# kwea123/ngp_pl

Measured on AMD Instinct MI355X. Metric: train rays/sec (800x800 Lego-like, 8192 rays/batch/GPU, full step incl. optimizer), higher is better.
Workload: dtype f16/f32

## Files before the change

### ngp_pl_amd/csrc/march.hip

```cpp
#pragma clang fp contract(off)

#include <cstdlib>
#include <chrono>
#include <type_traits>
#include "ngp_common.h"

#define NGP_SQRT3 1.73205080757f

namespace {

__device__ __forceinline__ float2 aabb_hit(float ox, float oy, float oz, float ix, float iy, float iz,
                                           float cx, float cy, float cz, float hx, float hy, float hz) {
    const float tminx = (cx - hx - ox) * ix, tmaxx = (cx + hx - ox) * ix;
    const float tminy = (cy - hy - oy) * iy, tmaxy = (cy + hy - oy) * iy;
    const float tminz = (cz - hz - oz) * iz, tmaxz = (cz + hz - oz) * iz;
    const float t1 = fmaxf(fmaxf(fminf(tminx, tmaxx), fminf(tminy, tmaxy)), fminf(tminz, tmaxz));
    const float t2 = fminf(fminf(fmaxf(tminx, tmaxx), fmaxf(tminy, tmaxy)), fmaxf(tminz, tmaxz));
    if (t1 > t2) return make_float2(-1.0f, -1.0f);
    return make_float2(t1, t2);
}

__device__ __forceinline__ float2 sphere_hit(float ox, float oy, float oz, float dx, float dy, float dz,
                                             float cx, float cy, float cz, float radius) {
    const float cox = ox - cx, coy = oy - cy, coz = oz - cz;
// ... 369 lines not shown
        int k = 1;
        const bool occ = march_probe<SIMPLE>(ray, p, mine, x, y, z, dt, t_next, &k);
        const unsigned long long empty_mask = ~__ballot(occ);
        int chain = occ ? ((lane << 8) | 64) : ((lane << 8) | (lane + k > 64 ? 64 : lane + k));
#pragma unroll 1
        for (int round = 0; round < 6; ++round) {
            const int h = chain & 0xff;
            const bool go = h < 64 && ((empty_mask >> h) & 1ull);
            const int via = __builtin_amdgcn_ds_bpermute((h & 63) << 2, chain);
            if (go) chain = via;
            if (!__ballot(go)) break;
        }
        unsigned long long emit = 0ull;
        float next_pending = -1.0f;
        bool finished = false;
        int v = entry;
        while (v < 64) {
            if (v >= nvalid) { finished = true; break; }
            if ((empty_mask >> v) & 1ull) {
                const int pk = __builtin_amdgcn_readlane(chain, v);
                const int h = pk & 0xff;
                if (h >= 64) {
                    next_pending = __builtin_bit_cast(float, __builtin_amdgcn_readlane(__builtin_bit_cast(int, t_next), pk >> 8));
                    v = 64;
                    break;
                }
                v = h;
                continue;
            }
            const unsigned long long un = empty_mask >> v;
            const int u = un ? v + (int)__builtin_ctzll(un) : 64;
            const int hi = u < nvalid ? u : nvalid;
            if (hi > v) {
                const int len = hi - v;
                emit |= (len >= 64 ? ~0ull : ((1ull << len) - 1ull)) << v;
            }
            if (nvalid < 64 && u >= nvalid) { finished = true; break; }
            v = u;
        }
        const int room = cap - n;
        const bool my = (emit >> lane) & 1ull;
        const int rank = __popcll(emit & ((1ull << lane) - 1ull));
        if (my && rank < room) store(n + rank, mine);
        const int cnt = __popcll(emit);
        n += cnt < room ? cnt : room;
        if (finished || n >= cap) break;
        pending = next_pending;
        if (pending >= 0 && !(pending < t2)) break;
        t_start = t_end;
    }
    return n;
}

struct MarchPrologue { const float* center; const float* half_size; float near_distance; uint32_t seed_lo, seed_hi; float* hits_out; float* noise_out; };
template <bool SIMPLE, bool PROLOGUE>
__global__ void __launch_bounds__(256)
march_train_count_wave_kernel(const float* __restrict__ rays_o, const float* __restrict__ rays_d,
                              const float* __restrict__ hits_t, const float* __restrict__ noise,
                              MarchParams p, int max_samples, int n_rays,
                              int64_t* __restrict__ rays_a, float* __restrict__ t_scratch, int32_t* __restrict__ counts, MarchPrologue pro) {
    const int r = __builtin_amdgcn_readfirstlane((int)((blockIdx.x * blockDim.x + threadIdx.x) >> 6));
    const int lane = threadIdx.x & 63;
    if (r >= n_rays) return;
    const Ray ray = load_ray(rays_o, rays_d, r);
    float t1, t2, jitter;
    if (PROLOGUE) {
        const float2 t = aabb_hit(ray.ox, ray.oy, ray.oz, ray.ix, ray.iy, ray.iz, pro.center[0], pro.center[1], pro.center[2],
                                  pro.half_size[0], pro.half_size[1], pro.half_size[2]);
        t1 = -1.0f; t2 = -1.0f;
        if (t.y > 0) { t1 = fmaxf(t.x, 0.0f); t2 = t.y; }
        if (t1 >= 0 && t1 < pro.near_distance) t1 = pro.near_distance;
        jitter = (float)(ngp_pcg_hash(ngp_rng_key(pro.seed_lo, pro.seed_hi, (uint32_t)r)) >> 8) * (1.0f / 16777216.0f);
        if (lane == 0) { reinterpret_cast<float2*>(pro.hits_out)[r] = make_float2(t1, t2); pro.noise_out[r] = jitter; }
    } else {
        t1 = hits_t[2 * r]; t2 = hits_t[2 * r + 1]; jitter = noise[r];
    }
    if (t1 >= 0) t1 = fmaf(calc_dt(t1, p), jitter, t1);
    float* __restrict__ row = t_scratch + (size_t)r * max_samples;
    int n = 0;
    if (t1 >= 0) n = march_tile_walk<SIMPLE>(ray, p, t1, t2, max_samples, lane, (unsigned int)r, [row](int i, float t) { row[i] = t; });
    if (lane == 0) {
        rays_a[3 * (size_t)r] = r;
        rays_a[3 * (size_t)r + 2] = n;
        if (counts) counts[r] = n;
    }
}

__global__ void __launch_bounds__(1024)
march_train_scan_kernel(int64_t* __restrict__ rays_a, int n_rays, int32_t* __restrict__ counter, int first_k, int32_t* __restrict__ offs_k) {
    __shared__ int s_wave[16], s_wave_k[16];
    __shared__ int s_carry, s_carry_k;
    const int tid = threadIdx.x;
    if (tid == 0) { s_carry = 0; s_carry_k = 0; }
    __syncthreads();
    for (int base = 0; base < n_rays; base += 8192) {
        const int r0 = base + 8 * tid;
        int v[8];
#pragma unroll
        for (int k = 0; k < 8; ++k) v[k] = (r0 + k < n_rays) ? (int)rays_a[3 * (size_t)(r0 + k) + 2] : 0;
        int run = ngp_block_scan_tile<8>(v, s_wave, &s_carry);
#pragma unroll
        for (int k = 0; k < 8; ++k) {
            if (r0 + k < n_rays) rays_a[3 * (size_t)(r0 + k) + 1] = run;
            run += v[k];
        }
        if (offs_k) {
            int vk[8];
#pragma unroll
            for (int k = 0; k < 8; ++k) vk[k] = min(v[k], first_k);
            int run_k = ngp_block_scan_tile<8>(vk, s_wave_k, &s_carry_k);
#pragma unroll
            for (int k = 0; k < 8; ++k) {
                if (r0 + k < n_rays) offs_k[r0 + k] = run_k;
                run_k += vk[k];
            }
        }
        __syncthreads();
    }
    if (tid == 0) { counter[0] = s_carry; counter[1] = n_rays; if (offs_k) counter[3] = s_carry_k; }
}

__global__ void __launch_bounds__(256)
march_train_write_kernel(const float* __restrict__ rays_o, const float* __restrict__ rays_d,
                         const int64_t* __restrict__ rays_a, const float* __restrict__ t_scratch,
                         MarchParams p, int max_samples, int n_rays,
                         float* __restrict__ xyzs, float* __restrict__ dirs,
                         float* __restrict__ deltas, float* __restrict__ ts,
                         int first_k, int32_t* __restrict__ list_k, int32_t* __restrict__ n_clear,
// ... 444 lines not shown
RenderLayout render_layout(int n_rays, int chunk_scale, float esf) {
    RenderLayout L;
    const int min_samples = (esf == 0.0f) ? 1 : 4;
    const long long R = n_rays;
    L.m_cap = R * (chunk_scale > min_samples ? chunk_scale : min_samples);
    size_t off = 0;
    auto take = [&](size_t bytes) { const size_t o = off; off += (bytes + 255) / 256 * 256; return o; };
    L.hits = take(R * 8); L.alive0 = take(R * 4); L.alive1 = take(R * 4); L.n_eff = take(R * 4); L.offsets = take(R * 4); L.emitted = take(R * 4);
    L.plan = take((RENDER_MAX_ITERS + 1) * sizeof(RenderPlan)); L.total = take(8); L.block_any = take(RENDER_MASK_WORDS * 4);
    const long long slack = 64;
    L.xyzs = take(L.m_cap * 12); L.dirs = take(L.m_cap * 12); L.deltas = take((L.m_cap + slack) * 4); L.ts = take((L.m_cap + slack) * 4);
    L.feats = take(L.m_cap * 64); L.sigmas = take((L.m_cap + slack) * 4); L.rgbs = take((L.m_cap + slack) * 12);
    L.bytes = off;
    return L;
}

struct RenderHost {
    int32_t* counts = nullptr;
    hipEvent_t ev[RENDER_RING] = {};
    int device = -1;
    int init() {
        int dev = 0;
        hipError_t e = hipGetDevice(&dev);
        if (e != hipSuccess) return (int)e;
        if (dev == device) return 0;
        if (device >= 0) {
            for (int i = 0; i < RENDER_RING; ++i) (void)hipEventDestroy(ev[i]);
            (void)hipHostFree(counts);
            device = -1;
        }
        e = hipHostMalloc(reinterpret_cast<void**>(&counts), RENDER_RING * sizeof(int32_t), hipHostMallocDefault);
        if (e != hipSuccess) return (int)e;
        for (int i = 0; i < RENDER_RING; ++i) {
            e = hipEventCreateWithFlags(&ev[i], hipEventDisableTiming);
            if (e != hipSuccess) return (int)e;
        }
        device = dev;
        return 0;
    }
};
thread_local RenderHost g_render_host;
static int g_render_block_hops = 1;
static int g_render_wave_rays = 80000;


double render_wait_limit_s() {
    static const double v = [] { const char* e = getenv("NGP_SPIN_TIMEOUT_S"); const double x = e ? atof(e) : 30.0; return x > 0 ? x : 30.0; }();
    return v;
}

template <typename F> void with_bool(bool flag, F f) { if (flag) f(std::true_type{}); else f(std::false_type{}); }

void launch_train_count(const float* rays_o, const float* rays_d, const float* hits_t, const float* noise, const MarchParams& p, int max_samples,
                        int n_rays, int64_t* rays_a, float* t_scratch, int32_t* counts, const MarchPrologue* pro, ngp_stream_t stream) {
    const dim3 grid(ngp_div_up((long long)n_rays * 64, 256));
    with_bool(p.simple, [&](auto S) { with_bool(pro != nullptr, [&](auto P) {
        hipLaunchKernelGGL((march_train_count_wave_kernel<decltype(S)::value, decltype(P)::value>), grid, dim3(256), 0, ngp_stream(stream),
                           rays_o, rays_d, hits_t, noise, p, max_samples, n_rays, rays_a, t_scratch, counts, pro ? *pro : MarchPrologue{});
    }); });
}

void launch_train_write(const float* rays_o, const float* rays_d, const int64_t* rays_a, const float* t_scratch, float scale, float exp_step_factor,
                        int grid_size, int max_samples, int n_rays, float* xyzs, float* dirs, float* deltas, float* ts,
                        int first_k, int32_t* list_k, int32_t* n_clear, const int32_t* offs_k,
                        const int32_t* counts, int64_t* rays_a_out, int32_t* counter, ngp_stream_t stream) {
    const MarchParams p = make_march_params(nullptr, 1, grid_size, scale, scale, exp_step_factor, max_samples);
    hipLaunchKernelGGL(march_train_write_kernel, dim3(ngp_div_up((long long)n_rays * 64, 256)), dim3(256), 0, ngp_stream(stream),
                       rays_o, rays_d, rays_a, t_scratch, p, max_samples, n_rays, xyzs, dirs, deltas, ts, first_k, list_k, n_clear, offs_k,
                       counts, rays_a_out, counter);
}

}

extern "C" {
#pragma GCC visibility push(default)

int ngp_abi_version(void) { return 6; }

int ngp_march_guard_first(float* probe12) {
    NGP_CHECK_PTR(probe12);
    return (int)hipMemcpyFromSymbol(probe12, HIP_SYMBOL(g_march_guard_first), 12 * sizeof(float), 0, hipMemcpyDeviceToHost);
}

int ngp_march_guard_read(uint32_t* counts4, int reset) {
    NGP_CHECK_PTR(counts4);
    hipError_t e = hipMemcpyFromSymbol(counts4, HIP_SYMBOL(g_march_guard), 4 * sizeof(uint32_t), 0, hipMemcpyDeviceToHost);
    if (e != hipSuccess) return (int)e;
    if (reset) {
        const uint32_t z[4] = {0, 0, 0, 0};
        e = hipMemcpyToSymbol(HIP_SYMBOL(g_march_guard), z, sizeof(z), 0, hipMemcpyHostToDevice);
    }
    return (int)e;
}
const char* ngp_build_arch(void) { return "gfx950"; }

int ngp_ray_aabb_intersect(const float* rays_o, const float* rays_d, const float* centers,
                           const float* half_sizes, int n_rays, int n_voxels, int max_hits,
                           int32_t* hit_cnt, float* hits_t, int64_t* hits_voxel_idx, ngp_stream_t stream) {
    if (n_rays < 0 || n_voxels < 0 || max_hits < 1) return NGP_EINVAL;
    if (n_rays == 0) return 0;
    NGP_CHECK_PTR(rays_o); NGP_CHECK_PTR(rays_d); NGP_CHECK_PTR(hit_cnt); NGP_CHECK_PTR(hits_t); NGP_CHECK_PTR(hits_voxel_idx);
    if (n_voxels > 0) { NGP_CHECK_PTR(centers); NGP_CHECK_PTR(half_sizes); }
    hipLaunchKernelGGL(ray_prim_intersect_kernel<false>, dim3(ngp_div_up(n_rays, 256)), dim3(256), 0, ngp_stream(stream),
                       rays_o, rays_d, centers, half_sizes, n_rays, n_voxels, max_hits, hit_cnt, hits_t, hits_voxel_idx);
    return NGP_LAUNCH_RESULT();
}

int ngp_ray_sphere_intersect(const float* rays_o, const float* rays_d, const float* centers,
                             const float* radii, int n_rays, int n_spheres, int max_hits,
                             int32_t* hit_cnt, float* hits_t, int64_t* hits_sphere_idx, ngp_stream_t stream) {
    if (n_rays < 0 || n_spheres < 0 || max_hits < 1) return NGP_EINVAL;
    if (n_rays == 0) return 0;
    NGP_CHECK_PTR(rays_o); NGP_CHECK_PTR(rays_d); NGP_CHECK_PTR(hit_cnt); NGP_CHECK_PTR(hits_t); NGP_CHECK_PTR(hits_sphere_idx);
    if (n_spheres > 0) { NGP_CHECK_PTR(centers); NGP_CHECK_PTR(radii); }
    hipLaunchKernelGGL(ray_prim_intersect_kernel<true>, dim3(ngp_div_up(n_rays, 256)), dim3(256), 0, ngp_stream(stream),
                       rays_o, rays_d, centers, radii, n_rays, n_spheres, max_hits, hit_cnt, hits_t, hits_sphere_idx);
    return NGP_LAUNCH_RESULT();
}

int ngp_ray_aabb_near(const float* rays_o, const float* rays_d, const float* center,
                      const float* half_size, float near_distance, int n_rays, float* hits_t,
                      ngp_stream_t stream) {
    if (n_rays < 0) return NGP_EINVAL;
    if (n_rays == 0) return 0;
// ... 67 lines not shown
                       density_grid, density_grid_tmp, decay_grid, decay, n_cells, stats);
    return NGP_LAUNCH_RESULT();
}

int ngp_raymarching_train_count(const float* rays_o, const float* rays_d, const float* hits_t,
                                const uint8_t* density_bitfield, int cascades, float scale,
                                float exp_step_factor, const float* noise, int grid_size,
                                int max_samples, int n_rays, int64_t* rays_a, int32_t* counter,
                                float* t_scratch, ngp_stream_t stream) {
    return ngp_raymarching_train_count_k(rays_o, rays_d, hits_t, density_bitfield, cascades, scale, exp_step_factor, noise, grid_size, max_samples,
                                         n_rays, rays_a, counter, t_scratch, 0, nullptr, stream);
}

int ngp_raymarching_train_count_k(const float* rays_o, const float* rays_d, const float* hits_t,
                                  const uint8_t* density_bitfield, int cascades, float scale,
                                  float exp_step_factor, const float* noise, int grid_size,
                                  int max_samples, int n_rays, int64_t* rays_a, int32_t* counter,
                                  float* t_scratch, int first_k, int32_t* offs_k, ngp_stream_t stream) {
    if (n_rays < 0 || cascades < 1 || grid_size < 1 || grid_size > 1024 || max_samples < 1) return NGP_EINVAL;
    if (offs_k != nullptr && (first_k < 1 || first_k > 64)) return NGP_EINVAL;
    NGP_CHECK_PTR(counter);
    if (n_rays > 0) {
        NGP_CHECK_PTR(rays_o); NGP_CHECK_PTR(rays_d); NGP_CHECK_PTR(hits_t); NGP_CHECK_PTR(density_bitfield);
        NGP_CHECK_PTR(noise); NGP_CHECK_PTR(rays_a); NGP_CHECK_PTR(t_scratch);
        const MarchParams p = make_march_params(density_bitfield, cascades, grid_size, scale, scale, exp_step_factor, max_samples);
        launch_train_count(rays_o, rays_d, hits_t, noise, p, max_samples, n_rays, rays_a, t_scratch, nullptr, nullptr, stream);
    }
    hipLaunchKernelGGL(march_train_scan_kernel, dim3(1), dim3(1024), 0, ngp_stream(stream), rays_a, n_rays, counter, first_k, offs_k);
    return NGP_LAUNCH_RESULT();
}

int ngp_raymarching_train_write(const float* rays_o, const float* rays_d, const int64_t* rays_a,
                                const float* t_scratch, float scale, float exp_step_factor,
                                int grid_size, int max_samples, int n_rays,
                                float* xyzs, float* dirs, float* deltas, float* ts, ngp_stream_t stream) {
    if (n_rays < 0 || grid_size < 1 || max_samples < 1) return NGP_EINVAL;
    if (n_rays == 0) return 0;
    NGP_CHECK_PTR(rays_o); NGP_CHECK_PTR(rays_d); NGP_CHECK_PTR(rays_a); NGP_CHECK_PTR(t_scratch);
    launch_train_write(rays_o, rays_d, rays_a, t_scratch, scale, exp_step_factor, grid_size, max_samples, n_rays, xyzs, dirs, deltas, ts,
                       0, nullptr, nullptr, nullptr, nullptr, nullptr, nullptr, stream);
    return NGP_LAUNCH_RESULT();
}

int ngp_march_train_fused(const float* rays_o, const float* rays_d, const float* center, const float* half_size,
                          float near_distance, uint64_t seed, const uint8_t* density_bitfield, int cascades, float scale,
                          float exp_step_factor, int grid_size, int max_samples, int n_rays,
                          float* hits_t, float* noise, int64_t* rays_a, int32_t* counts, int32_t* counter, float* t_scratch,
                          float* xyzs, float* dirs, float* deltas, float* ts, ngp_stream_t stream) {
    if (n_rays < 1 || cascades < 1 || grid_size < 1 || grid_size > 1024 || max_samples < 1) return NGP_EINVAL;
    NGP_CHECK_PTR(rays_o); NGP_CHECK_PTR(rays_d); NGP_CHECK_PTR(center); NGP_CHECK_PTR(half_size); NGP_CHECK_PTR(density_bitfield);
    NGP_CHECK_PTR(hits_t); NGP_CHECK_PTR(noise); NGP_CHECK_PTR(rays_a); NGP_CHECK_PTR(counts); NGP_CHECK_PTR(counter); NGP_CHECK_PTR(t_scratch);
    NGP_CHECK_PTR(xyzs); NGP_CHECK_PTR(dirs); NGP_CHECK_PTR(deltas); NGP_CHECK_PTR(ts);
    if (reinterpret_cast<uintptr_t>(counts) & 15) return NGP_EINVAL;
    const MarchParams p = make_march_params(density_bitfield, cascades, grid_size, scale, scale, exp_step_factor, max_samples);
    const MarchPrologue pro = {center, half_size, near_distance, (uint32_t)seed, (uint32_t)(seed >> 32), hits_t, noise};
    launch_train_count(rays_o, rays_d, nullptr, nullptr, p, max_samples, n_rays, rays_a, t_scratch, counts, &pro, stream);
    launch_train_write(rays_o, rays_d, rays_a, t_scratch, scale, exp_step_factor, grid_size, max_samples, n_rays, xyzs, dirs, deltas, ts,
                       0, nullptr, nullptr, nullptr, counts, rays_a, counter, stream);
    return NGP_LAUNCH_RESULT();
}

int ngp_raymarching_train_write_k(const float* rays_o, const float* rays_d, const int64_t* rays_a,
                                  const float* t_scratch, float scale, float exp_step_factor,
                                  int grid_size, int max_samples, int n_rays,
                                  float* xyzs, float* dirs, float* deltas, float* ts,
                                  int first_k, int32_t* list_k, int32_t* n_clear, ngp_stream_t stream) {
    if (n_rays < 0 || grid_size < 1 || max_samples < 1 || first_k < 1 || first_k > 64) return NGP_EINVAL;
    if (n_rays == 0) return 0;
    NGP_CHECK_PTR(rays_o); NGP_CHECK_PTR(rays_d); NGP_CHECK_PTR(rays_a); NGP_CHECK_PTR(t_scratch); NGP_CHECK_PTR(list_k);
    launch_train_write(rays_o, rays_d, rays_a, t_scratch, scale, exp_step_factor, grid_size, max_samples, n_rays, xyzs, dirs, deltas, ts,
                       first_k, list_k, n_clear, nullptr, nullptr, nullptr, nullptr, stream);
    return NGP_LAUNCH_RESULT();
}

int ngp_raymarching_train_write_kc(const float* rays_o, const float* rays_d, const int64_t* rays_a,
                                   const float* t_scratch, float scale, float exp_step_factor,
                                   int grid_size, int max_samples, int n_rays,
                                   float* xyzs, float* dirs, float* deltas, float* ts,
                                   int first_k, const int32_t* offs_k, int32_t* list_k, int32_t* n_clear, ngp_stream_t stream) {
    if (n_rays < 0 || grid_size < 1 || max_samples < 1 || first_k < 1 || first_k > 64) return NGP_EINVAL;
    if (n_rays == 0) return 0;
    NGP_CHECK_PTR(rays_o); NGP_CHECK_PTR(rays_d); NGP_CHECK_PTR(rays_a); NGP_CHECK_PTR(t_scratch); NGP_CHECK_PTR(list_k); NGP_CHECK_PTR(offs_k);
    launch_train_write(rays_o, rays_d, rays_a, t_scratch, scale, exp_step_factor, grid_size, max_samples, n_rays, xyzs, dirs, deltas, ts,
                       first_k, list_k, n_clear, offs_k, nullptr, nullptr, nullptr, stream);
    return NGP_LAUNCH_RESULT();
}

int ngp_raymarching_test(const float* rays_o, const float* rays_d, float* hits_t,
                         const int64_t* alive_indices, const uint8_t* density_bitfield,
                         int cascades, float scale, float exp_step_factor, int grid_size,
                         int max_samples, int n_samples, int n_alive,
                         float* xyzs, float* dirs, float* deltas, float* ts,
                         int32_t* n_eff_samples, ngp_stream_t stream) {
    if (n_alive < 0 || cascades < 1 || grid_size < 1 || grid_size > 1024 || max_samples < 1 || n_samples < 1) return NGP_EINVAL;
    if (n_alive == 0) return 0;
    NGP_CHECK_PTR(rays_o); NGP_CHECK_PTR(rays_d); NGP_CHECK_PTR(hits_t); NGP_CHECK_PTR(alive_indices);
    NGP_CHECK_PTR(density_bitfield); NGP_CHECK_PTR(xyzs); NGP_CHECK_PTR(dirs); NGP_CHECK_PTR(deltas);
    NGP_CHECK_PTR(ts); NGP_CHECK_PTR(n_eff_samples);
    const MarchParams p = make_march_params(density_bitfield, cascades, grid_size, scale, (float)cascades, exp_step_factor, max_samples);
    with_bool(p.simple, [&](auto S) {
        hipLaunchKernelGGL(march_test_kernel<decltype(S)::value>, dim3(ngp_div_up(n_alive, 64)), dim3(64), 0, ngp_stream(stream),
                           rays_o, rays_d, hits_t, alive_indices, p, n_samples, n_alive, xyzs, dirs, deltas, ts, n_eff_samples);
    });
    return NGP_LAUNCH_RESULT();
}

int ngp_compact_alive(const int64_t* alive_in, const int32_t* n_eff, int n, int64_t* alive_out, int32_t* count,
                      int64_t* total_samples, ngp_stream_t stream) {
    if (n < 0) return NGP_EINVAL;
    if (n == 0) return 0;
    NGP_CHECK_PTR(alive_in); NGP_CHECK_PTR(alive_out); NGP_CHECK_PTR(count);
    hipLaunchKernelGGL(compact_alive_kernel, dim3(ngp_div_up(n, 256)), dim3(256), 0, ngp_stream(stream),
// ... 132 lines not shown
```

### ngp_pl_amd/csrc/ngp_internal.h

```cpp
#ifndef NGP_HIP_INTERNAL_H
#define NGP_HIP_INTERNAL_H
#include "../../include/ngp_hip.h"
#ifdef __cplusplus
extern "C" {
#endif

typedef struct ngp_grid_partials {
    int32_t n_levels, reserved;
    int64_t value_end;
    uint32_t offset[NGP_MAX_LEVELS + 1];
    int32_t k_split[NGP_MAX_LEVELS];
    int64_t part_off[NGP_MAX_LEVELS];
    const float* partial;
} ngp_grid_partials;

int ngp_field_bwd_guarded(const ngp_half* feats, const float* dirs, const ngp_half* h, const ngp_half* density_w,
                          const ngp_half* rgb_w, const float* dL_dsigmas, const float* dL_drgbs, float loss_scale,
                          const float* loss_scale_dev, float din_limit, int n_samples, const int32_t* active_idx, const int32_t* n_active,
                          ngp_half* dh_scratch, ngp_half* dfeats, float* wgrad_partial, int32_t* nonfinite2, int parity,
                          ngp_stream_t stream);
int ngp_adam_use_loss_scaler(float* state, int slot, float growth_factor, float backoff_factor, int growth_interval,
                             float min_scale, float max_scale);
struct ngp_stepper;
int ngp_stepper_before_update(struct ngp_stepper* s, int32_t** found_inf);
// ... 89 lines not shown
int ngp_composite_train_bw_tail(const float* dL_dopacity, const float* dL_ddepth, const float* dL_drgb,
                                const float* dL_dws, const float* sigmas, const float* rgbs, const float* ws,
                                const float* deltas, const float* ts, const int64_t* rays_a,
                                const float* opacity, const float* depth, const float* rgb, float T_threshold,
                                int n_rays, int n_samples, float* dL_dsigmas, float* dL_drgbs,
                                const int32_t* ray_counts, int32_t* active_idx, const float* xyzs, float* x_active,
                                int32_t* n_active, int32_t* n_active_host, float* loss, float* sq_err,
                                const void* workspace, size_t workspace_bytes, ngp_stream_t stream);

int ngp_hashgrid_fwd_list(const float* x, const float* xyz_min, const float* xyz_max,
                          const ngp_half* table, const ngp_grid_meta* meta, int n_samples,
                          const int32_t* list, int n_list_max, const int32_t* n_list_dev,
                          ngp_half* feats, ngp_stream_t stream);

int ngp_field_fwd_list(const ngp_half* feats, const float* dirs,
                       const ngp_half* density_w, const ngp_half* rgb_w, int n_samples,
                       const int32_t* list, int n_list_max, const int32_t* n_list_dev,
                       float* sigmas, float* rgbs, ngp_half* h_out, ngp_stream_t stream);

int ngp_density_fwd_scatter(const ngp_half* feats, const ngp_half* density_w, int n_samples,
                            const int32_t* scatter_idx, float* sigmas_out, ngp_stream_t stream);

int ngp_debug_hashgrid_fwd_map(const ngp_grid_meta* meta, int n_chunks, int32_t* xcd_level_chunk, int max_blocks);

int ngp_debug_render_block_hops(int enabled);

int ngp_debug_render_wave_rays(int max_rays);

int ngp_stepper_two_rounds(const ngp_stepper* s);

int ngp_occupancy_update_workspace_layout(int cascades, int grid_size, size_t* tmp_off, size_t* cell_idx_off, size_t* xyzs_off);

int ngp_feats_to_rowmajor(const ngp_half* feats, int n_levels, int n_samples, ngp_half* out,
                          ngp_stream_t stream);

int ngp_feats_from_rowmajor(const ngp_half* in, int n_levels, int n_samples, ngp_half* feats,
                            ngp_stream_t stream);

int ngp_adam_step_partials(float* param, ngp_half* param_h, const float* partials, int n_partials,
                           float* m, float* v, int n, float lr, float beta1, float beta2, float eps,
                           float weight_decay, int step, float grad_scale, const int32_t* found_inf,
                           ngp_stream_t stream);

int ngp_active_samples(const int64_t* rays_a, const int64_t* total_samples, int n_rays,
                       int32_t* ray_offsets, int32_t* active_idx, int32_t* n_active,
                       ngp_stream_t stream);

int ngp_hashgrid_bwd(const float* x, const float* xyz_min, const float* xyz_max,
                     const ngp_half* dfeats , const ngp_grid_meta* meta,
                     int n_samples, void* grad_table, int grad_is_f32, ngp_stream_t stream);

#ifdef __cplusplus
}
#endif
#endif
```

### ngp_pl_amd/csrc/stepper.hip

```cpp
#include "ngp_common.h"
#include "adam_common.h"
#include "comm.h"
#include <algorithm>
#include <chrono>
#include <cstdlib>
#include <cstring>
#include <new>

namespace {

constexpr int N_MARKS = 9;

double spin_limit_s() {
    static const double v = [] { const char* e = getenv("NGP_SPIN_TIMEOUT_S"); const double x = e ? atof(e) : 30.0; return x > 0 ? x : 30.0; }();
    return v;
}

}

struct ngp_stepper {
    ngp_stepper_config c;
    ngp_step_buffers b;
    hipEvent_t ready[2] = {}, done[2] = {};
    hipEvent_t mark[N_MARKS] = {}, march_t[2][2] = {};
    bool mark_set[N_MARKS] = {}, march_t_set[2] = {};
    int timing = 0;
    int next_set = 0;
    bool has_pending = false;
    const float* pend_o = nullptr; const float* pend_d = nullptr;
    int pend_set = 0;
    uint64_t marches = 0;
    int32_t S = 0, n_part = 0, last_set = 0;
    bool binned = false;
    int device = 0;
    double t_wait = 0.0, t_enqueue = 0.0;
    long long n_fronts = 0;
    const float* next_o = nullptr; const float* next_d = nullptr;
    hipStream_t next_main = nullptr, next_side = nullptr;
    int march_at = 2;
    int two_round_mode = 2, two_round_k = 32;
    bool two_round_active = false, two_rounds = false;
    int set_k[2] = {0, 0};
    long long two_round_steps = 0;
    int32_t prev_S = 0;
    ngp_comm* comm = nullptr;
    ngp_exchange_config x = {};
    hipEvent_t ev_small = nullptr, ev_chunk[8] = {}, ev_done = nullptr;
    hipEvent_t ev_x0 = nullptr, ev_x1 = nullptr, ev_m = nullptr;
    bool x_times_set = false;
    long long tails = 0;
    int64_t group_end[16] = {};
    struct SampleSet { float* xyzs; float* dirs; float* deltas; float* ts; };
    SampleSet samples[2] = {};
    bool two_sample_sets = false;
    bool expanded[2] = {false, false};
    int32_t* counts[2] = {nullptr, nullptr};
    int counts_rays = 0;
    bool same_stream[2] = {false, false};
    int32_t* guard = nullptr;
    int guard_parity = 0;
    bool guard_armed = false;
    bool fused[2] = {false, false};
    float* scaler_state = nullptr;
    bool scaler_on = false;
    int scaler_slot = 0;
    float scaler_growth = 2.0f, scaler_backoff = 0.5f, scaler_lo = 9.5367431640625e-07f , scaler_hi = 1.152921504606847e18f ;
    int scaler_interval = 2000;
};

void destroy_exchange_events(ngp_stepper* s);

namespace {

struct HostTimer {
    double* acc; std::chrono::steady_clock::time_point t0;
    explicit HostTimer(double* a) : acc(a), t0(std::chrono::steady_clock::now()) {}
    ~HostTimer() { *acc += std::chrono::duration<double>(std::chrono::steady_clock::now() - t0).count(); }
};

#define STEP_TRY(expr) do { const int rc_ = (expr); if (rc_ != 0) return rc_; } while (0)
#define STEP_HIP(expr) do { const hipError_t e_ = (expr); if (e_ != hipSuccess) return (int)e_; } while (0)

int check_buffers(const ngp_stepper_config& c, const ngp_step_buffers& b) {
    if (b.n_rays < 1 || b.cap < b.n_rays || b.max_partials < 1) return NGP_EINVAL;
    const void* need[] = {b.xyzs, b.dirs, b.deltas, b.ts, b.feats, b.h, b.sigmas, b.rgbs, b.ws, b.dL_dsigmas, b.dL_drgbs, b.active, b.dh,
                          b.dfeats, b.total, b.opacity, b.depth, b.rgb, b.dL_drgb, b.dL_dopacity, b.ray_offs, b.zeros, b.n_active, b.stats,
                          b.partials, b.fw_ws, b.hits_t[0], b.hits_t[1], b.rays_a[0], b.rays_a[1], b.noise[0], b.noise[1], b.scratch[0],
                          b.scratch[1], b.counter[0], b.counter[1]};
    for (const void* p : need) if (p == nullptr) return NGP_EINVAL;
    if (b.bin_max > 0 && (b.bin_ws == nullptr || b.x_act == nullptr)) return NGP_EINVAL;
    if (b.distortion && (!b.ws_incl || !b.wts_incl || !b.dL_dws || !b.dist || !b.dist_seed)) return NGP_EINVAL;
    if (c.lambda_distortion > 0 && !b.distortion) return NGP_EINVAL;
    return 0;
}

inline void mark(ngp_stepper* s, int i, hipStream_t st) {
    if (!s->timing) return;
    if (hipEventRecord(s->mark[i], st) == hipSuccess) s->mark_set[i] = true;
}

int wait_march(ngp_stepper* s, int k, bool count_is_enough = false) {
    volatile int32_t* cnt = s->b.counter[k];
    const auto t_begin = std::chrono::steady_clock::now();
    struct Account { ngp_stepper* s; std::chrono::steady_clock::time_point t0;
                     ~Account() { const double d = std::chrono::duration<double>(std::chrono::steady_clock::now() - t0).count(); s->t_wait += d; s->t_enqueue -= d; } } account{s, t_begin};
    const auto t_end = t_begin + std::chrono::duration<double>(spin_limit_s());
    unsigned spins = 0;
    while (cnt[0] < 0) {
        if ((++spins & 1023u) == 0) {
            if (hipEventQuery(s->done[k]) == hipSuccess) break;
// ... 10 lines not shown

enum { AT_TOP = 0, AT_HASHGRID_FWD, AT_MLP_FWD, AT_COMPOSITE_FW, AT_COMPOSITE_BW, AT_MLP_BWD, AT_HASHGRID_BWD, AT_ADAM };
int march_at_from_env() {
    static const int v = [] {
        const char* e = getenv("NGP_MARCH_AT");
        if (!e) return (int)AT_MLP_FWD;
        const char* names[] = {"top", "hashgrid_fwd", "mlp_fwd", "composite_fw", "composite_bw", "mlp_bwd", "hashgrid_bwd", "adam"};
        for (int i = 0; i < 8; ++i) if (strcmp(e, names[i]) == 0) return i;
        return (int)AT_MLP_FWD;
    }();
    return v;
}

int ensure_counts(ngp_stepper* s) {
    const int n = s->b.n_rays;
    if (s->counts[0] != nullptr && s->counts_rays >= n) return 0;
    for (int k = 0; k < 2; ++k) { if (s->counts[k]) (void)hipFree(s->counts[k]); s->counts[k] = nullptr; }
    for (int k = 0; k < 2; ++k) STEP_HIP(hipMalloc(reinterpret_cast<void**>(&s->counts[k]), ((size_t)n + 8) * sizeof(int32_t)));
    s->counts_rays = n;
    return 0;
}

int do_march(ngp_stepper* s, const float* rays_o, const float* rays_d, hipStream_t main, hipStream_t side);
inline int march_next_if_at(ngp_stepper* s, int stage) {
    if (s->next_o == nullptr || s->march_at != stage) return 0;
    const float* o = s->next_o; const float* d = s->next_d;
    s->next_o = s->next_d = nullptr;
    return do_march(s, o, d, s->next_main, s->next_side);
}

int do_march(ngp_stepper* s, const float* rays_o, const float* rays_d, hipStream_t main, hipStream_t side) {
    if (s->has_pending) return NGP_EINVAL;
    NGP_CHECK_PTR(rays_o); NGP_CHECK_PTR(rays_d);
    const ngp_stepper_config& c = s->c;
    const ngp_step_buffers& b = s->b;
    const int k = s->next_set; s->next_set ^= 1;
    if (side != main) {
        STEP_HIP(hipEventRecord(s->ready[k], main));
        STEP_HIP(hipStreamWaitEvent(side, s->ready[k], 0));
    }
    b.counter[k][0] = -1;
    b.counter[k][3] = -1;
    s->march_t_set[k] = false;
    s->same_stream[k] = side == main;
    s->fused[k] = false;
    if (s->timing) STEP_HIP(hipEventRecord(s->march_t[k][0], side));
    const bool lists_wanted = (s->two_round_mode == 1 || (s->two_round_mode == 2 && s->two_round_active)) && b.list_k && b.list_rest &&
                              b.two_round_counts && b.offs_k[k];
    constexpr int FUSED_MARCH_MAX_RAYS = 32768;
    if (s->two_sample_sets && !lists_wanted && b.n_rays <= FUSED_MARCH_MAX_RAYS) {
        STEP_TRY(ensure_counts(s));
        const ngp_stepper::SampleSet& w = s->samples[k];
        s->set_k[k] = 0;
        STEP_TRY(ngp_march_train_fused(rays_o, rays_d, c.center, c.half_size, c.near_distance, c.noise_seed + 0x9E3779B97F4A7C15ull * (++s->marches),
                                       c.density_bitfield, c.cascades, c.scale, c.exp_step_factor, c.grid_size, c.max_samples, b.n_rays,
                                       b.hits_t[k], b.noise[k], b.rays_a[k], s->counts[k], b.counter[k], b.scratch[k],
                                       w.xyzs, w.dirs, w.deltas, w.ts, (ngp_stream_t)side));
        s->expanded[k] = true;
        s->fused[k] = true;
        if (s->timing) { STEP_HIP(hipEventRecord(s->march_t[k][1], side)); s->march_t_set[k] = true; }
        STEP_HIP(hipEventRecord(s->done[k], side));
        s->has_pending = true; s->pend_o = rays_o; s->pend_d = rays_d; s->pend_set = k;
        return 0;
    }
    STEP_TRY(ngp_ray_aabb_near_noise(rays_o, rays_d, c.center, c.half_size, c.near_distance, b.n_rays, c.noise_seed + 0x9E3779B97F4A7C15ull * (++s->marches),
                                     b.hits_t[k], b.noise[k], (ngp_stream_t)side));
    const bool lists = (s->two_round_mode == 1 || (s->two_round_mode == 2 && s->two_round_active)) && b.list_k && b.list_rest &&
                       b.two_round_counts && b.offs_k[k];
    s->set_k[k] = lists ? s->two_round_k : 0;
    STEP_TRY(ngp_raymarching_train_count_k(rays_o, rays_d, b.hits_t[k], c.density_bitfield, c.cascades, c.scale, c.exp_step_factor, b.noise[k],
                                           c.grid_size, c.max_samples, b.n_rays, b.rays_a[k], b.counter[k], b.scratch[k], s->set_k[k],
                                           lists ? b.offs_k[k] : nullptr, (ngp_stream_t)side));
    s->expanded[k] = false;
    if (s->two_sample_sets && side != main && !lists) {
        const ngp_stepper::SampleSet& w = s->samples[k];
        STEP_TRY(ngp_raymarching_train_write(rays_o, rays_d, b.rays_a[k], b.scratch[k], c.scale, c.exp_step_factor, c.grid_size, c.max_samples, b.n_rays,
                                             w.xyzs, w.dirs, w.deltas, w.ts, (ngp_stream_t)side));
        s->expanded[k] = true;
    }
    if (s->timing) { STEP_HIP(hipEventRecord(s->march_t[k][1], side)); s->march_t_set[k] = true; }
    STEP_HIP(hipEventRecord(s->done[k], side));
    s->has_pending = true; s->pend_o = rays_o; s->pend_d = rays_d; s->pend_set = k;
    return 0;
}

}

void destroy_exchange_events(ngp_stepper* s) {
    hipEvent_t* all[] = {&s->ev_small, &s->ev_done, &s->ev_x0, &s->ev_x1, &s->ev_m};
    for (hipEvent_t* e : all) if (*e) { (void)hipEventDestroy(*e); *e = nullptr; }
    for (int i = 0; i < 8; ++i) if (s->ev_chunk[i]) { (void)hipEventDestroy(s->ev_chunk[i]); s->ev_chunk[i] = nullptr; }
}

extern "C" {
#pragma GCC visibility push(default)

int ngp_stepper_create(const ngp_stepper_config* config, const ngp_step_buffers* buffers, ngp_stepper** out) {
    if (!config || !buffers || !out) return NGP_EINVAL;
    *out = nullptr;
    const ngp_stepper_config& c = *config;
    const void* need[] = {c.center, c.half_size, c.xyz_min, c.xyz_max, c.density_bitfield, c.enc_half, c.rgb_half, c.grid_grad16};
    for (const void* p : need) if (p == nullptr) return NGP_EINVAL;
    if (c.cascades < 1 || c.grid_size < 1 || c.max_samples < 1 || c.n_grid < 1 || c.n_density != NGP_DENSITY_NET_PARAMS || c.n_rgb != NGP_RGB_NET_PARAMS)
        return NGP_EINVAL;
    if (c.meta.n_features != 2 || c.meta.n_levels != 16) return NGP_EUNSUP;
    const int rc = check_buffers(c, *buffers);
    if (rc) return rc;
    ngp_stepper* s = new (std::nothrow) ngp_stepper();
    if (!s) return NGP_EINVAL;
    s->c = c; s->b = *buffers;
    s->march_at = march_at_from_env();
    if (const char* e = getenv("NGP_TWO_ROUND")) s->two_round_mode = strcmp(e, "on") == 0 ? 1 : (strcmp(e, "off") == 0 ? 0 : 2);
    if (const char* e = getenv("NGP_TWO_ROUND_K")) { const int k = atoi(e); if (k >= 1 && k <= 64) s->two_round_k = k; }
    (void)hipGetDevice(&s->device);
    hipError_t e = hipSuccess;
    for (int k = 0; k < 2 && e == hipSuccess; ++k) {
        e = hipEventCreateWithFlags(&s->ready[k], hipEventDisableTiming);
        if (e == hipSuccess) e = hipEventCreateWithFlags(&s->done[k], hipEventDisableTiming);
        for (int j = 0; j < 2 && e == hipSuccess; ++j) e = hipEventCreate(&s->march_t[k][j]);
    }
    for (int i = 0; i < N_MARKS && e == hipSuccess; ++i) e = hipEventCreate(&s->mark[i]);
    if (e == hipSuccess) e = hipMalloc(reinterpret_cast<void**>(&s->guard), 2 * sizeof(int32_t));
    if (e == hipSuccess) e = hipMemset(s->guard, 0, 2 * sizeof(int32_t));
    if (e == hipSuccess) e = hipMalloc(reinterpret_cast<void**>(&s->scaler_state), 4 * sizeof(float));
    if (e != hipSuccess) { ngp_stepper_destroy(s); return (int)e; }
    *out = s;
    return 0;
}

int ngp_stepper_destroy(ngp_stepper* s) {
    if (!s) return 0;
    if (s->has_pending) (void)wait_march(s, s->pend_set);
    for (int k = 0; k < 2; ++k) {
        if (s->ready[k]) (void)hipEventDestroy(s->ready[k]);
        if (s->done[k]) (void)hipEventDestroy(s->done[k]);
        for (int j = 0; j < 2; ++j) if (s->march_t[k][j]) (void)hipEventDestroy(s->march_t[k][j]);
    }
    for (int i = 0; i < N_MARKS; ++i) if (s->mark[i]) (void)hipEventDestroy(s->mark[i]);
    for (int k = 0; k < 2; ++k) if (s->counts[k]) (void)hipFree(s->counts[k]);
    if (s->guard) (void)hipFree(s->guard);
    if (s->scaler_state) (void)hipFree(s->scaler_state);
    destroy_exchange_events(s);
    delete s;
    return 0;
}

int ngp_stepper_drop_pending(ngp_stepper* s) {
    if (!s) return NGP_EINVAL;
    if (!s->has_pending) return 0;
    const int rc = wait_march(s, s->pend_set);
    s->next_set = s->pend_set;
    s->has_pending = false;
    return rc;
}

int ngp_stepper_set_buffers(ngp_stepper* s, const ngp_step_buffers* buffers) {
    if (!s || !buffers) return NGP_EINVAL;
    STEP_TRY(ngp_stepper_drop_pending(s));
    STEP_TRY(check_buffers(s->c, *buffers));
    s->b = *buffers;
    s->two_sample_sets = false; s->expanded[0] = s->expanded[1] = false;
    s->S = 0; s->n_part = 0;
    s->set_k[0] = s->set_k[1] = 0;
    s->two_round_active = false; s->two_rounds = false;
    s->prev_S = 0;
    return 0;
}

int ngp_stepper_set_sample_sets(ngp_stepper* s, float* xyzs1, float* dirs1, float* deltas1, float* ts1) {
    if (!s) return NGP_EINVAL;
    STEP_TRY(ngp_stepper_drop_pending(s));
    const bool all = xyzs1 && dirs1 && deltas1 && ts1, none = !xyzs1 && !dirs1 && !deltas1 && !ts1;
    if (!all && !none) return NGP_EINVAL;
    if (s->two_sample_sets) {
        s->b.xyzs = s->samples[0].xyzs; s->b.dirs = s->samples[0].dirs; s->b.deltas = s->samples[0].deltas; s->b.ts = s->samples[0].ts;
    }
    s->expanded[0] = s->expanded[1] = false;
    s->two_sample_sets = all;
    if (all) {
        NGP_CHECK_PTR(xyzs1); NGP_CHECK_PTR(dirs1); NGP_CHECK_PTR(deltas1); NGP_CHECK_PTR(ts1);
        s->samples[0] = {s->b.xyzs, s->b.dirs, s->b.deltas, s->b.ts};
        s->samples[1] = {xyzs1, dirs1, deltas1, ts1};
    }
    return 0;
}

int ngp_stepper_pending(const ngp_stepper* s, const float* rays_o, const float* rays_d) {
    return (s && s->has_pending && s->pend_o == rays_o && s->pend_d == rays_d) ? 1 : 0;
}

int ngp_stepper_last_set(const ngp_stepper* s) { return s ? s->last_set : 0; }
int ngp_stepper_two_rounds(const ngp_stepper* s) { return (s && s->two_rounds) ? 1 : 0; }
int ngp_stepper_record_bytes(int which) {
    return which == 0 ? (int)sizeof(ngp_stepper_config) : which == 1 ? (int)sizeof(ngp_step_buffers) : which == 2 ? (int)sizeof(ngp_exchange_config) : NGP_EINVAL;
// ... 528 lines not shown
```

Measured before the change: 24.20 million.

## Prune ray far bound using coarse dilated occupancy reach table before marching

Adds a small kernel that reduces the 128^3 density bitfield to a 16^3 coarse occupancy map plus a 3x3x3-dilated reach map. In the simple single-cascade path, each ray wave samples up to 64 points along its AABB segment against the reach map and shrinks t2 to just past the last reachable block, or drops the ray entirely if no coarse block is occupied. The aim is to stop the tile walk from scanning empty space beyond the object. It costs one extra tiny kernel launch per march and a ballot pre-pass per ray, and relies on the dilation being conservative enough that no occupied cells are skipped.

```diff
diff --git a/ngp_pl_amd/csrc/march.hip b/ngp_pl_amd/csrc/march.hip
--- a/ngp_pl_amd/csrc/march.hip
+++ b/ngp_pl_amd/csrc/march.hip
@@ -445,13 +445,67 @@
     return n;
 }
 
+constexpr int REACH_WORDS = 128;
+__global__ void __launch_bounds__(256)
+march_reach_table_kernel(const uint8_t* __restrict__ bitfield, uint32_t* __restrict__ any_out, uint32_t* __restrict__ reach_out) {
+    __shared__ uint32_t s_col[256];
+    const int tid = threadIdx.x, lane = tid & 63;
+    const int bx = tid & 15, by = tid >> 4, bz = blockIdx.x;
+    uint4 v[3][4];
+#pragma unroll
+    for (int k = 0; k < 3; ++k) {
+        const uint32_t b = ngp_morton3D((uint32_t)bx, (uint32_t)by, (uint32_t)min(max(bz + k - 1, 0), 15));
+        const uint4* cells = reinterpret_cast<const uint4*>(bitfield) + 4 * (size_t)b;
+#pragma unroll
+        for (int i = 0; i < 4; ++i) v[k][i] = cells[i];
+    }
+    uint32_t o[3];
+#pragma unroll
+    for (int k = 0; k < 3; ++k) {
+        o[k] = 0u;
+#pragma unroll
+        for (int i = 0; i < 4; ++i) o[k] |= v[k][i].x | v[k][i].y | v[k][i].z | v[k][i].w;
+    }
+    const int l = (bz << 8) | tid;
+    const unsigned long long m_any = __ballot(o[1] != 0u);
+    if (lane == 0) { any_out[l >> 5] = (uint32_t)m_any; any_out[(l >> 5) + 1] = (uint32_t)(m_any >> 32); }
+    s_col[tid] = o[0] | o[1] | o[2];
+    __syncthreads();
+    uint32_t r = 0u;
+#pragma unroll
+    for (int dy = -1; dy <= 1; ++dy)
+#pragma unroll
+        for (int dx = -1; dx <= 1; ++dx) r |= s_col[(min(max(by + dy, 0), 15) << 4) | min(max(bx + dx, 0), 15)];
+    const unsigned long long m = __ballot(r != 0u);
+    if (lane == 0) { reach_out[l >> 5] = (uint32_t)m; reach_out[(l >> 5) + 1] = (uint32_t)(m >> 32); }
+}
+
+__device__ __forceinline__ float march_reach_far(const Ray& ray, const MarchParams& p, const uint32_t* __restrict__ reach, float t1, float t2, int lane) {
+    const float step = (p.bound0 * 0.0625f) / sqrtf(ray.dx * ray.dx + ray.dy * ray.dy + ray.dz * ray.dz);
+    const float q = (t2 - t1) / step;
+    const float mag = fabsf(ray.ox) + fabsf(ray.oy) + fabsf(ray.oz) + fabsf(ray.dx) + fabsf(ray.dy) + fabsf(ray.dz) + t2;
+    if (!(step > 0.0f && step < 3.0e38f && q >= 0.0f && q < 61.0f && mag < 3.0e38f)) return t2;
+    const int need = (int)q + 2;
+    const float t = fmaf((float)lane, step, t1);
+    const float x = fmaf(t, ray.dx, ray.ox), y = fmaf(t, ray.dy, ray.oy), z = fmaf(t, ray.dz, ray.oz);
+    const int bx = (int)fmaxf(0.0f, fminf(0.5f * (x * p.bound0_inv + 1) * 16.0f, 15.0f));
+    const int by = (int)fmaxf(0.0f, fminf(0.5f * (y * p.bound0_inv + 1) * 16.0f, 15.0f));
+    const int bz = (int)fmaxf(0.0f, fminf(0.5f * (z * p.bound0_inv + 1) * 16.0f, 15.0f));
+    const int l = (bz << 8) | (by << 4) | bx;
+    const unsigned long long m = __ballot(lane < need && ((reach[l >> 5] >> (l & 31)) & 1u) != 0u);
+    if (!m) return -1.0f;
+    const int last = 63 - (int)__builtin_clzll(m);
+    return fminf(t2, fmaf((float)(last + 1), step, t1));
+}
+
 struct MarchPrologue { const float* center; const float* half_size; float near_distance; uint32_t seed_lo, seed_hi; float* hits_out; float* noise_out; };
 template <bool SIMPLE, bool PROLOGUE>
 __global__ void __launch_bounds__(256)
 march_train_count_wave_kernel(const float* __restrict__ rays_o, const float* __restrict__ rays_d,
                               const float* __restrict__ hits_t, const float* __restrict__ noise,
                               MarchParams p, int max_samples, int n_rays,
-                              int64_t* __restrict__ rays_a, float* __restrict__ t_scratch, int32_t* __restrict__ counts, MarchPrologue pro) {
+                              int64_t* __restrict__ rays_a, float* __restrict__ t_scratch, int32_t* __restrict__ counts, MarchPrologue pro,
+                              const uint32_t* __restrict__ reach) {
     const int r = __builtin_amdgcn_readfirstlane((int)((blockIdx.x * blockDim.x + threadIdx.x) >> 6));
     const int lane = threadIdx.x & 63;
     if (r >= n_rays) return;
@@ -467,6 +521,10 @@
         if (lane == 0) { reinterpret_cast<float2*>(pro.hits_out)[r] = make_float2(t1, t2); pro.noise_out[r] = jitter; }
     } else {
         t1 = hits_t[2 * r]; t2 = hits_t[2 * r + 1]; jitter = noise[r];
+    }
+    if (SIMPLE && reach != nullptr && t1 >= 0) {
+        t2 = march_reach_far(ray, p, reach, t1, t2, lane);
+        if (t2 < 0) t1 = -1.0f;
     }
     if (t1 >= 0) t1 = fmaf(calc_dt(t1, p), jitter, t1);
     float* __restrict__ row = t_scratch + (size_t)r * max_samples;
@@ -1017,11 +1075,12 @@
 template <typename F> void with_bool(bool flag, F f) { if (flag) f(std::true_type{}); else f(std::false_type{}); }
 
 void launch_train_count(const float* rays_o, const float* rays_d, const float* hits_t, const float* noise, const MarchParams& p, int max_samples,
-                        int n_rays, int64_t* rays_a, float* t_scratch, int32_t* counts, const MarchPrologue* pro, ngp_stream_t stream) {
+                        int n_rays, int64_t* rays_a, float* t_scratch, int32_t* counts, const MarchPrologue* pro, ngp_stream_t stream,
+                        const uint32_t* reach = nullptr) {
     const dim3 grid(ngp_div_up((long long)n_rays * 64, 256));
     with_bool(p.simple, [&](auto S) { with_bool(pro != nullptr, [&](auto P) {
         hipLaunchKernelGGL((march_train_count_wave_kernel<decltype(S)::value, decltype(P)::value>), grid, dim3(256), 0, ngp_stream(stream),
-                           rays_o, rays_d, hits_t, noise, p, max_samples, n_rays, rays_a, t_scratch, counts, pro ? *pro : MarchPrologue{});
+                           rays_o, rays_d, hits_t, noise, p, max_samples, n_rays, rays_a, t_scratch, counts, pro ? *pro : MarchPrologue{}, reach);
     }); });
 }
 
@@ -1035,6 +1094,24 @@
                        counts, rays_a_out, counter);
 }
 
+}
+
+int march_train_fused_reach(const float* rays_o, const float* rays_d, const float* center, const float* half_size,
+                            float near_distance, uint64_t seed, const uint8_t* density_bitfield, int cascades, float scale,
+                            float exp_step_factor, int grid_size, int max_samples, int n_rays,
+                            float* hits_t, float* noise, int64_t* rays_a, int32_t* counts, int32_t* counter, float* t_scratch,
+                            float* xyzs, float* dirs, float* deltas, float* ts, uint32_t* reach_ws, ngp_stream_t stream) {
+    const MarchParams p = make_march_params(density_bitfield, cascades, grid_size, scale, scale, exp_step_factor, max_samples);
+    const MarchPrologue pro = {center, half_size, near_distance, (uint32_t)seed, (uint32_t)(seed >> 32), hits_t, noise};
+    const uint32_t* reach = nullptr;
+    if (reach_ws != nullptr && p.simple && grid_size == 128 && (reinterpret_cast<uintptr_t>(density_bitfield) & 15) == 0) {
+        hipLaunchKernelGGL(march_reach_table_kernel, dim3(16), dim3(256), 0, ngp_stream(stream), density_bitfield, reach_ws, reach_ws + REACH_WORDS);
+        reach = reach_ws + REACH_WORDS;
+    }
+    launch_train_count(rays_o, rays_d, nullptr, nullptr, p, max_samples, n_rays, rays_a, t_scratch, counts, &pro, stream, reach);
+    launch_train_write(rays_o, rays_d, rays_a, t_scratch, scale, exp_step_factor, grid_size, max_samples, n_rays, xyzs, dirs, deltas, ts,
+                       0, nullptr, nullptr, nullptr, counts, rays_a, counter, stream);
+    return NGP_LAUNCH_RESULT();
 }
 
 extern "C" {
@@ -1208,12 +1285,9 @@
     NGP_CHECK_PTR(hits_t); NGP_CHECK_PTR(noise); NGP_CHECK_PTR(rays_a); NGP_CHECK_PTR(counts); NGP_CHECK_PTR(counter); NGP_CHECK_PTR(t_scratch);
     NGP_CHECK_PTR(xyzs); NGP_CHECK_PTR(dirs); NGP_CHECK_PTR(deltas); NGP_CHECK_PTR(ts);
     if (reinterpret_cast<uintptr_t>(counts) & 15) return NGP_EINVAL;
-    const MarchParams p = make_march_params(density_bitfield, cascades, grid_size, scale, scale, exp_step_factor, max_samples);
-    const MarchPrologue pro = {center, half_size, near_distance, (uint32_t)seed, (uint32_t)(seed >> 32), hits_t, noise};
-    launch_train_count(rays_o, rays_d, nullptr, nullptr, p, max_samples, n_rays, rays_a, t_scratch, counts, &pro, stream);
-    launch_train_write(rays_o, rays_d, rays_a, t_scratch, scale, exp_step_factor, grid_size, max_samples, n_rays, xyzs, dirs, deltas, ts,
-                       0, nullptr, nullptr, nullptr, counts, rays_a, counter, stream);
-    return NGP_LAUNCH_RESULT();
+    return march_train_fused_reach(rays_o, rays_d, center, half_size, near_distance, seed, density_bitfield, cascades, scale, exp_step_factor,
+                                   grid_size, max_samples, n_rays, hits_t, noise, rays_a, counts, counter, t_scratch, xyzs, dirs, deltas, ts,
+                                   nullptr, stream);
 }
 
 int ngp_raymarching_train_write_k(const float* rays_o, const float* rays_d, const int64_t* rays_a,
diff --git a/ngp_pl_amd/csrc/ngp_internal.h b/ngp_pl_amd/csrc/ngp_internal.h
--- a/ngp_pl_amd/csrc/ngp_internal.h
+++ b/ngp_pl_amd/csrc/ngp_internal.h
@@ -165,5 +165,11 @@
 
 #ifdef __cplusplus
 }
+__attribute__((visibility("hidden")))
+int march_train_fused_reach(const float* rays_o, const float* rays_d, const float* center, const float* half_size,
+                            float near_distance, uint64_t seed, const uint8_t* density_bitfield, int cascades, float scale,
+                            float exp_step_factor, int grid_size, int max_samples, int n_rays,
+                            float* hits_t, float* noise, int64_t* rays_a, int32_t* counts, int32_t* counter, float* t_scratch,
+                            float* xyzs, float* dirs, float* deltas, float* ts, uint32_t* reach_ws, ngp_stream_t stream);
 #endif
 #endif
diff --git a/ngp_pl_amd/csrc/stepper.hip b/ngp_pl_amd/csrc/stepper.hip
--- a/ngp_pl_amd/csrc/stepper.hip
+++ b/ngp_pl_amd/csrc/stepper.hip
@@ -56,6 +56,7 @@
     bool expanded[2] = {false, false};
     int32_t* counts[2] = {nullptr, nullptr};
     int counts_rays = 0;
+    uint32_t* reach_ws = nullptr;
     bool same_stream[2] = {false, false};
     int32_t* guard = nullptr;
     int guard_parity = 0;
@@ -172,10 +173,11 @@
         STEP_TRY(ensure_counts(s));
         const ngp_stepper::SampleSet& w = s->samples[k];
         s->set_k[k] = 0;
-        STEP_TRY(ngp_march_train_fused(rays_o, rays_d, c.center, c.half_size, c.near_distance, c.noise_seed + 0x9E3779B97F4A7C15ull * (++s->marches),
-                                       c.density_bitfield, c.cascades, c.scale, c.exp_step_factor, c.grid_size, c.max_samples, b.n_rays,
-                                       b.hits_t[k], b.noise[k], b.rays_a[k], s->counts[k], b.counter[k], b.scratch[k],
-                                       w.xyzs, w.dirs, w.deltas, w.ts, (ngp_stream_t)side));
+        const bool simple = c.cascades == 1 && c.exp_step_factor == 0.0f;
+        STEP_TRY(march_train_fused_reach(rays_o, rays_d, c.center, c.half_size, c.near_distance, c.noise_seed + 0x9E3779B97F4A7C15ull * (++s->marches),
+                                         c.density_bitfield, c.cascades, c.scale, c.exp_step_factor, c.grid_size, c.max_samples, b.n_rays,
+                                         b.hits_t[k], b.noise[k], b.rays_a[k], s->counts[k], b.counter[k], b.scratch[k],
+                                         w.xyzs, w.dirs, w.deltas, w.ts, simple ? s->reach_ws : nullptr, (ngp_stream_t)side));
         s->expanded[k] = true;
         s->fused[k] = true;
         if (s->timing) { STEP_HIP(hipEventRecord(s->march_t[k][1], side)); s->march_t_set[k] = true; }
@@ -243,6 +245,8 @@
     if (e == hipSuccess) e = hipMalloc(reinterpret_cast<void**>(&s->guard), 2 * sizeof(int32_t));
     if (e == hipSuccess) e = hipMemset(s->guard, 0, 2 * sizeof(int32_t));
     if (e == hipSuccess) e = hipMalloc(reinterpret_cast<void**>(&s->scaler_state), 4 * sizeof(float));
+    const char* prune = getenv("NGP_MARCH_PRUNE");
+    if (e == hipSuccess && !(prune && strcmp(prune, "0") == 0)) e = hipMalloc(reinterpret_cast<void**>(&s->reach_ws), 256 * sizeof(uint32_t));
     if (e != hipSuccess) { ngp_stepper_destroy(s); return (int)e; }
     *out = s;
     return 0;
@@ -260,6 +264,7 @@
     for (int k = 0; k < 2; ++k) if (s->counts[k]) (void)hipFree(s->counts[k]);
     if (s->guard) (void)hipFree(s->guard);
     if (s->scaler_state) (void)hipFree(s->scaler_state);
+    if (s->reach_ws) (void)hipFree(s->reach_ws);
     destroy_exchange_events(s);
     delete s;
     return 0;
```

Measured after the change: 24.50 million, median of 6. 1.2% higher.
